# MiloszKrajewski/lz4net

Measured on AMD Instinct MI355X. Metric: uncompressed GB/s, batched 64KiB-block encode+decode: value = decode (known output size) per step over the whole resident batch; fast encode and LZ4HC encode of the same data in roofline_encode / roofline_hc, higher is better.
Workload: dtype u8

## Files before the change

### lz4net_amd/csrc/lz4hip_decode_lane4.hpp

```cpp
#pragma once
#include "lz4hip_common.hpp"
#include <type_traits>

#ifndef LZ4HIP_ITERATION_HOOK
#define LZ4HIP_ITERATION_HOOK(lane) ((void)0)
#endif
#ifndef LZ4HIP_STAT
#define LZ4HIP_STAT(slot, cond) ((void)0)
#endif
#ifdef LZ4HIP_SECTION_MARKERS
#define LZ4HIP_SECTION(name) asm volatile("; @@SECTION " name)
#else
#define LZ4HIP_SECTION(name) ((void)0)
#endif

namespace lz4hip {

#ifndef LZ4HIP_DEC4_FLUSH_RECS
#define LZ4HIP_DEC4_FLUSH_RECS 0
#endif
#ifndef LZ4HIP_DEC4_DUAL_STORE
#define LZ4HIP_DEC4_DUAL_STORE 2
#endif
constexpr unsigned lane4_lds_bytes(int ring_bytes) { return 64u * (unsigned)ring_bytes + 16u * 32u; }

struct NoNext {
    static constexpr bool kPersistent = false;
    LZ4HIP_DEVICE bool operator()(int, const uint8_t*&, int&, uint8_t*&, int&) const { return false; }
};

enum L4Kind { kK4None = 0, kK4Near = 1, kK4Far = 2, kK4Lit = 3, kK4Zero = 4 };
enum L4Flag { kF4Final = 1, kF4Err = 2, kF4Header = 4 };

template <bool KNOWN, int R, int P, int FU, int FS, int FE = 1, int IE = 1, int POL = 0, class NEXT = NoNext, int WAVES = 1>
LZ4HIP_DEVICE int lane4_decode_block(unsigned char* lds, int lane, bool active, const uint8_t* src, int iend,
                                     uint8_t* dst, int oend, NEXT next = NEXT(), int wave = 0)
{
    static_assert(WAVES == 1 || WAVES == 4, "one or four wavefronts per workgroup");
    constexpr uint32_t kRow = 256u * (uint32_t)WAVES;
    static_assert(R >= 128 && R % 16 == 0 && R <= 1008, "ring: a multiple of 16 bytes, 128 .. 1008");
    static_assert(P == 32 || P == 64, "input piece: 32 or 64 bytes");
    static_assert(FU == 64 || (FU == 128 && R >= 192), "flush unit: 64 bytes, or 128 with a ring of at least 192");
    static_assert(FS == 1 || FS == 2, "one or two flush store instructions per iteration");
    static_assert(FE == 1 || FE == 2, "the flush runs in every iteration or in every second one");
    static_assert(IE == 1 || (IE == 2 && FE == 2), "input requests in every iteration, or alternating with the flush");
    constexpr int RW = R / 4;
    constexpr bool RPOW2 = (RW & (RW - 1)) == 0;
    constexpr uint32_t kRingBytes = (uint32_t)RW * kRow;
    constexpr uint32_t kLdsBytes = lane4_lds_bytes(R) * (uint32_t)WAVES;
    constexpr bool LS = (POL & 16) != 0;
    constexpr int kDual = (POL & 32) ? 0 : (LZ4HIP_DEC4_DUAL_STORE);
    static_assert(!LS || P == 32, "sector input feeds 32-byte pieces");
    constexpr int SK = LS ? 64 : P;
    constexpr int NW = 4 + P / 4, NL = LS ? 4 : P / 16;
    constexpr int HPR = FU / 16, RECS_PER_STORE = 64 / HPR;
    constexpr int kFlushRecs = (LZ4HIP_DEC4_FLUSH_RECS) ? (LZ4HIP_DEC4_FLUSH_RECS) : FS * RECS_PER_STORE;
    constexpr bool kLineNoWrap = R % 64 == 0;
    constexpr int kNearMax = R - 20;
    unsigned char* const frec_base = lds + kRingBytes + (uint32_t)wave * 256u;
    auto frec = [&](int i) -> Aligned16* {
        if (kFlushRecs <= 16) return (Aligned16*)(frec_base + (uint32_t)i * 16u);
        return (Aligned16*)(frec_base + (uint32_t)(i >> 4) * kRow + (uint32_t)(i & 15) * 16u);
    };
    const uint32_t lane4 = (uint32_t)(wave * 64 + lane) << 2;

    auto ring_add = [](uint32_t a, uint32_t rows256) -> uint32_t {
        const uint32_t t = a + rows256;
        if (RPOW2) return t & (kRingBytes - 1u);
        const uint32_t u = t - kRingBytes;
        return u < t ? u : t;
    };
#define L4_RING(a) (*(uint32_t*)(lds + (a)))
#define L4_PHASE_SEL(p_) wv::alignbyte(0x07060504u, 0x03020100u, (uint32_t)(p_) & 3u)

    int skew = 0, in_total = 0;
    uint64_t src_al = 0;
    uint32_t out_limit = 0;
    int ip = 0;
    uint32_t W[NW];
    wv::u32x4 L[NL];
    int wb = -16;
    int lvalid = 0;
    int pend_a = 0, pend_b = 0;
    int op = 0, fl = 0;
    uint32_t oa = lane4;
    int kind = kK4None, rem = 0, off = 8;
    int gready = 0;
    int pv = 0, p_ll = 0, p_st = 0, p_ml = 0, p_off = 0, p_flags = 0, p_res = 0;
    uint32_t p_l0 = 0, p_l1 = 0, p_l2 = 0;
    int hdr = 0;
    uint32_t token = 0;
    int final_seen = 0, final_run = 0, result = 0, done = 0;
    int exhausted = 0;
    wv::u32x4 fa = { 0, 0, 0, 0 }, fb = { 0, 0, 0, 0 };
#if defined(LZ4HIP_DEC4_BALLAST_VALU) || defined(LZ4HIP_DEC4_BALLAST_LDS)
    uint32_t ballast = 0;
#endif
#pragma unroll
    for (int j = 0; j < NW; j++) W[j] = 0;
#pragma unroll
    for (int j = 0; j < NL; j++) L[j] = wv::u32x4{ 0, 0, 0, 0 };
    auto start_block = [&](bool act) {
        skew = (int)((uint64_t)src & (uint64_t)(SK - 1));
        src_al = (uint64_t)src - (uint64_t)skew;
        in_total = iend > 0 ? (int)(((int64_t)skew + iend + P - 1) & ~(int64_t)(P - 1)) : 0;
        out_limit = oend > kLastLiterals ? (uint32_t)(oend - kLastLiterals) : 0u;
        ip = 0; wb = -16 - P; lvalid = 0; pend_a = 0; pend_b = 0; op = 0; fl = 0; oa = lane4;
        kind = kK4None; rem = 0; off = 8; gready = 0;
        pv = 0; p_ll = 0; p_st = 0; p_ml = 0; p_off = 0; p_flags = 0; p_res = 0; hdr = 0; token = 0;
        final_seen = 0; final_run = 0; result = 0; done = 0;
        if (!act || (!KNOWN && iend == 0)) { done = 1; final_seen = 1; }
    };
    start_block(active);

#define L4_STORE2(OFF_, v_) do { const uint32_t w_ = (v_); wv::lds_store_drop<OFF_>(lds, kLdsBytes, oa, w_); wv::lds_store_drop<OFF_>(lds, kLdsBytes, ob_, w_); } while (0)
#define L4_APPEND(d0_, d1_, d2_, d3_, n_, FOUR_)                                                         \
    do {                                                                                                \
        const uint32_t sb_ = (uint32_t)op & 3u;                                                         \
        const uint32_t s_ = wv::alignbyte(0x08070605u, 0x04030201u, sb_ ^ 3u);                          \
        wv::lds_mskor(&L4_RING(oa), 0xFFFFFFFFu << (8u * sb_), wv::perm(d0_, 0u, s_));                  \
        if (kDual) {                                                                                    \
                                                    \
            const uint32_t ob_ = oa - kRingBytes;                                                       \
            const uint32_t w1_ = wv::perm(d1_, d0_, s_), w2_ = wv::perm(d2_, d1_, s_);                  \
            if (kDual == 2) {                                         \
                wv::lds_store2_rows_drop<1 * WAVES, 2 * WAVES>(lds, kLdsBytes, oa, w1_, w2_);           \
                wv::lds_store2_rows_drop<1 * WAVES, 2 * WAVES>(lds, kLdsBytes, ob_, w1_, w2_);          \
                if (FOUR_) {                                                                            \
                    const uint32_t w3_ = wv::perm(d3_, d2_, s_), w4_ = wv::perm(0u, d3_, s_);           \
                    wv::lds_store2_rows_drop<3 * WAVES, 4 * WAVES>(lds, kLdsBytes, oa, w3_, w4_);       \
                    wv::lds_store2_rows_drop<3 * WAVES, 4 * WAVES>(lds, kLdsBytes, ob_, w3_, w4_);      \
                } else {                                                                                \
                    L4_STORE2(3 * kRow, wv::perm(0u, d2_, s_));                                         \
                }                                                                                       \
            } else {                                                                                    \
                L4_STORE2(kRow, w1_);                                                                   \
                L4_STORE2(2 * kRow, w2_);                                                               \
                if (FOUR_) {                                                                            \
                    L4_STORE2(3 * kRow, wv::perm(d3_, d2_, s_));                                        \
                    L4_STORE2(4 * kRow, wv::perm(0u, d3_, s_));                                         \
                } else {                                                                                \
                    L4_STORE2(3 * kRow, wv::perm(0u, d2_, s_));                                         \
                }                                                                                       \
            }                                                                                           \
        } else {                                                                                        \
            const uint32_t a1_ = ring_add(oa, kRow), a2_ = ring_add(oa, 2 * kRow), a3_ = ring_add(oa, 3 * kRow); \
            L4_RING(a1_) = wv::perm(d1_, d0_, s_);                                                      \
            L4_RING(a2_) = wv::perm(d2_, d1_, s_);                                                      \
            if (FOUR_) {                                                                                \
                L4_RING(a3_) = wv::perm(d3_, d2_, s_);                                                  \
                L4_RING(ring_add(oa, 4 * kRow)) = wv::perm(0u, d3_, s_);                                \
            } else {                                                                                    \
                L4_RING(a3_) = wv::perm(0u, d2_, s_);                                                   \
            }                                                                                           \
        }                                                                                               \
        oa = ring_add(oa, (((sb_ + (uint32_t)(n_)) << 6) & 0x700u) * (uint32_t)WAVES);                  \
        op += (n_);                                                                                     \
    } while (0)

    auto iteration = [&](auto flush_tag, wv::u32x4& ldF, wv::u32x4& usF, int& ld_pend, int& us_pend) __attribute__((always_inline)) -> bool {
        constexpr bool FLUSH = decltype(flush_tag)::value;
        constexpr bool INPUT = IE == 1 || !FLUSH;
        constexpr int kVm = (FLUSH ? FS : 0) + 1 + (INPUT ? NL : 0);
        LZ4HIP_ITERATION_HOOK(lane);
        LZ4HIP_SECTION("T1a window refill");
        int d = ip + skew - wb;
        {
            const bool no_more = wb + 16 + P >= in_total;
            const bool cross = (d >= P) & ((lvalid != 0) | no_more);
            const wv::mask_t cm = wv::cond(d >= P) & (wv::cond(lvalid != 0) | wv::cond(no_more));
#pragma unroll
            for (int j = 0; j < 4; j++) W[j] = wv::sel(cm, W[P / 4 + j], W[j]);
            if constexpr (LS) {
                const bool hi_half = ((wb + 16 + P) & 32) != 0;
                const wv::mask_t hm = wv::cond(((wb + 16 + P) & 32) != 0);
#pragma unroll
                for (int j = 0; j < 2; j++) {
                    W[4 + 4 * j] = wv::sel(cm, wv::sel(hm, L[2 + j].x, L[j].x), W[4 + 4 * j]); W[5 + 4 * j] = wv::sel(cm, wv::sel(hm, L[2 + j].y, L[j].y), W[5 + 4 * j]);
                    W[6 + 4 * j] = wv::sel(cm, wv::sel(hm, L[2 + j].z, L[j].z), W[6 + 4 * j]); W[7 + 4 * j] = wv::sel(cm, wv::sel(hm, L[2 + j].w, L[j].w), W[7 + 4 * j]);
                }
                lvalid = (cross & hi_half) ? 0 : lvalid;
            } else {
#pragma unroll
                for (int j = 0; j < NL; j++) {
                    W[4 + 4 * j] = wv::sel(cm, L[j].x, W[4 + 4 * j]); W[5 + 4 * j] = wv::sel(cm, L[j].y, W[5 + 4 * j]);
                    W[6 + 4 * j] = wv::sel(cm, L[j].z, W[6 + 4 * j]); W[7 + 4 * j] = wv::sel(cm, L[j].w, W[7 + 4 * j]);
                }
                lvalid = cross ? 0 : lvalid;
            }
            wb += cross ? P : 0;
            d -= cross ? P : 0;
        }
        LZ4HIP_SECTION("T1b cursor view (select tree + rotation)");
        const bool staged16 = d < P;
        LZ4HIP_STAT(0, true); LZ4HIP_STAT(1, done == 0); LZ4HIP_STAT(2, (done == 0) & !staged16);
        uint32_t x0, x1, x2, x3;
        {
            const uint32_t k = (uint32_t)d >> 2;
            uint32_t t[NW];
#pragma unroll
            for (int j = 0; j < NW; j++) t[j] = W[j];
            int n = NW;
#pragma unroll
            for (int sh = P / 8; sh >= 1; sh >>= 1) {
                const wv::mask_t m = wv::cond((k & (uint32_t)sh) != 0u);
                n -= sh;
#pragma unroll
                for (int j = 0; j < NW; j++)
                    if (j < n) t[j] = wv::sel(m, t[j + sh], t[j]);
            }
            const uint32_t sx = L4_PHASE_SEL(d);
            x0 = wv::perm(t[1], t[0], sx); x1 = wv::perm(t[2], t[1], sx); x2 = wv::perm(t[3], t[2], sx); x3 = wv::perm(t[4], t[3], sx);
        }
        LZ4HIP_SECTION("T1c near-match source rows");
        uint32_t v0, v1, v2, v3;
        {
            const uint32_t offn = kind == kK4Near ? (uint32_t)off : 4u;
            const uint32_t back = (((offn + 3u - ((uint32_t)op & 3u)) << 6) & ~0xFFu) * (uint32_t)WAVES;
            uint32_t sa;
            if (RPOW2) sa = (oa - back) & (kRingBytes - 1u);
            else { const uint32_t t = oa - back, u = t + kRingBytes; sa = u < t ? u : t; }
            const uint32_t r0 = L4_RING(sa), r1 = L4_RING(ring_add(sa, kRow)), r2 = L4_RING(ring_add(sa, 2 * kRow)),
                           r3 = L4_RING(ring_add(sa, 3 * kRow)), r4 = L4_RING(ring_add(sa, 4 * kRow));
            const uint32_t sr = L4_PHASE_SEL((uint32_t)op - offn);
            v0 = wv::perm(r1, r0, sr); v1 = wv::perm(r2, r1, sr); v2 = wv::perm(r3, r2, sr); v3 = wv::perm(r4, r3, sr);
        }

        LZ4HIP_SECTION("T2 cooperative flush");
        if constexpr (FLUSH) {
            const bool need = (done == 0) & (op - fl >= FU);
            const uint64_t needy = wv::ballot(need);
            const int cnt_all = wv::popc64(needy);
            const bool go = cnt_all != 0;
            int cnt = 0;
            bool mine = false;
            if (go) {
                cnt = cnt_all < kFlushRecs ? cnt_all : kFlushRecs;
                const int frank = wv::rank_below(needy);
                mine = need & (frank < kFlushRecs);
                if (mine) {
                    const uint64_t dp = (uint64_t)dst;
                    *frec(frank) = Aligned16{ { ring_add(oa, kRingBytes - ((((uint32_t)(op - fl)) << 6) & ~0xFFu) * (uint32_t)WAVES), (uint32_t)fl, (uint32_t)dp, (uint32_t)(dp >> 32) } };
                }
                wv::mem_sync();
            }
            const int sub = lane % HPR;
#pragma unroll
            for (int base = 0; base < FS * RECS_PER_STORE; base += RECS_PER_STORE) {
                const int idx = base + lane / HPR;
                const bool act = idx < cnt;
                const wv::mask_t act_m = wv::cond(idx < cnt);
                uint64_t g = 0;
                uint32_t q0 = 0, q1 = 0, q2 = 0, q3 = 0;
                if (act) {
                    const Aligned16 r = *frec(idx);
                    g = ((uint64_t)r.w[2] | ((uint64_t)r.w[3] << 32)) + (uint64_t)(r.w[1] + 16u * (uint32_t)sub);
                    const uint32_t b0 = ring_add(r.w[0], 4u * kRow * (uint32_t)sub);
                    if (kLineNoWrap) { q0 = L4_RING(b0); q1 = L4_RING(b0 + kRow); q2 = L4_RING(b0 + 2 * kRow); q3 = L4_RING(b0 + 3 * kRow); }
                    else { q0 = L4_RING(b0); q1 = L4_RING(ring_add(b0, kRow)); q2 = L4_RING(ring_add(b0, 2 * kRow)); q3 = L4_RING(ring_add(b0, 3 * kRow)); }
                }
                wv::vm_store16_mask(act_m, g, q0, q1, q2, q3);
            }
            LZ4HIP_STAT(3, need); LZ4HIP_STAT(4, need & !mine);
            if (go) {
                wv::mem_sync();
                fl += mine ? FU : 0;
            }
        }
        LZ4HIP_SECTION("T3 chunk size");
        const bool room = op - fl <= R - 46;
        const bool near = kind == kK4Near, lit = kind == kK4Lit;
        const bool can = room & (rem > 0) & !((kind == kK4Far) & (gready == 0)) & !(lit & !staged16);
        const int stride = (near & (off < 16)) ? off : 16;
        int n = can ? (rem < stride ? rem : stride) : 0;
        n = ((kind == kK4Zero) & (n > 8)) ? 8 : n;
        LZ4HIP_STAT(5, (done == 0) & (rem > 0)); LZ4HIP_STAT(6, (done == 0) & (rem > 0) & (n == 0)); LZ4HIP_STAT(7, (done == 0) & (rem > 0) & !room);
        LZ4HIP_STAT(8, (done == 0) & (rem > 0) & (kind == kK4Far) & (gready == 0)); LZ4HIP_STAT(9, (done == 0) & (rem > n));
        const int rem_after = rem - n;
        const int op_end = op + rem;

        LZ4HIP_SECTION("T4 parse ahead");
        const bool may_parse = (pv == 0) & (final_seen == 0) & !(lit & (rem > 0)) & staged16;
        LZ4HIP_STAT(10, may_parse); LZ4HIP_STAT(11, (done == 0) & (pv != 0));
        if (may_parse) {
            const uint32_t tok = hdr ? token : (x0 & 255u);
            const uint32_t t4 = tok >> 4, b1 = (x0 >> 8) & 255u, mlc = tok & 15u;
            const bool e1 = (hdr == 0) & (t4 == 15u), e2 = mlc == 15u;
            const int ll = hdr ? 0 : (int)t4 + (e1 ? (int)b1 : 0);
            const bool in_win = (hdr != 0) | (t4 <= 11u);
            const int o = hdr ? 0 : 1 + (int)t4;
            uint32_t ot;
            {
                const uint32_t q = (uint32_t)o >> 2;
                const wv::mask_t m1 = wv::cond((q & 1u) != 0u), m2 = wv::cond((q & 2u) != 0u);
                const uint32_t lo = wv::sel(m2, wv::sel(m1, x3, x2), wv::sel(m1, x1, x0));
                const uint32_t hi = wv::sel(m2, x3, wv::sel(m1, x2, x1));
                ot = wv::alignbyte(hi, lo, (uint32_t)o & 3u);
            }
            const int vo = (int)(ot & 0xFFFFu);
            const uint32_t extb = (ot >> 16) & 255u;
            const int ml = (int)mlc + kMinMatch + (e2 ? (int)extb : 0);
            const int lit_end = op_end + ll;
            const int p_after = ip + o + 2;
            bool trap = (ip + 16 > iend) | (e1 & (b1 == 255u)) | (ip + 1 + (e1 ? 1 : 0) + ll > iend);
            trap |= in_win & ((e2 & (extb == 255u)) | (vo > lit_end) | ((uint32_t)lit_end + (uint32_t)ml > out_limit));
            if (KNOWN) trap |= (hdr == 0) & (lit_end > oend - 8);
            else       trap |= ((hdr == 0) & ((lit_end > oend - kMfLimit) | (ip + 1 + (e1 ? 1 : 0) + ll > iend - 8))) | (in_win & e2 & !(p_after < iend - (kLastLiterals + 1)));
            p_l0 = wv::alignbyte(x1, x0, 1); p_l1 = wv::alignbyte(x2, x1, 1); p_l2 = wv::alignbyte(x3, x2, 1);
            token = tok;
            p_ll = in_win ? ll : 0;
            p_st = in_win ? 0 : ll;
            p_ml = in_win ? ml : 0;
            p_off = vo;
            p_flags = in_win ? 0 : (int)kF4Header;
            const int ip_fast = in_win ? p_after + (e2 ? 1 : 0) : ip + 1 + (e1 ? 1 : 0);
            if (trap) {
                LZ4HIP_SECTION("T4x byte-wise parser (trap)");
                int err = 0, pos = ip;
                if (!hdr) {
                    const uint32_t tk = ip < iend ? src[ip] : 0u;
                    int l = (int)(tk >> 4);
                    pos = ip + 1;
                    if (l == 15) {
                        uint32_t b = 255;
                        if (KNOWN) { do { b = pos < iend ? src[pos] : 0u; pos++; l += (int)b; if (l > (1 << 30)) { err = -pos; l = 0; break; } } while (b == 255); }
                        else       { while (pos < iend && b == 255) { b = src[pos]; pos++; l += (int)b; l = l > (1 << 30) ? (1 << 30) : l; } }
                    }
                    token = tk;
                    const int le = (int)((int64_t)op_end + l > 0x7FFFFFFF ? 0x7FFFFFFF : op_end + l);
                    const bool last = KNOWN ? (le > oend - 8) : ((le > oend - kMfLimit) | (pos + l > iend - 8));
                    p_ll = 0; p_st = l; p_ml = 0; p_off = 8;
                    if (last) {
                        if (KNOWN) { if (err == 0 && (le != oend || pos + l > iend)) err = -pos; }
                        else       { if (le > oend || pos + l != iend) err = -pos; }
                        p_flags = kF4Final;
                        p_res = KNOWN ? pos + l : le;
                        final_seen = 1;
                    } else {
                        if (KNOWN && err == 0 && pos + l > iend) err = -pos;
                        p_flags = kF4Header;
                    }
                    ip = pos;
                } else {
                    int p = ip;
                    const int o_ = (int)((p < iend ? src[p] : 0u) | ((p + 1 < iend ? src[p + 1] : 0u) << 8));
                    p += 2;
                    int m = (int)(token & 15u);
                    if (m == 15) {
                        if (KNOWN) {
                            uint32_t b;
                            while ((b = (p < iend ? src[p] : 0u)) == 255) { m += 255; p++; if (m > (1 << 30)) { err = -p; break; } }
                            m += (int)b; p++;
                        } else {
                            while (p < iend - (kLastLiterals + 1)) { const uint32_t b = src[p]; p++; m += (int)b; m = m > (1 << 30) ? (1 << 30) : m; if (b != 255) break; }
                        }
                    }
                    m += kMinMatch;
                    if (err != 0) {}
                    else if (op_end - o_ < 0) err = -(ip + 2);
                    else if ((int64_t)op_end + m > (int64_t)oend - kLastLiterals) err = -p;
                    p_ll = 0; p_st = 0; p_ml = m; p_off = o_; p_flags = 0;
                    ip = p;
                    hdr = 0;
                }
                if (err != 0) { p_flags = kF4Err; p_res = err; }
                hdr = (p_flags & kF4Header) ? 1 : 0;
            } else {
                ip = ip_fast;
                hdr = in_win ? 0 : 1;
            }
            LZ4HIP_SECTION("T4 parse ahead");
            pv = 1;
        }

        LZ4HIP_SECTION("T5 far fetch");
        {
            const wv::mask_t m_rem0 = wv::cond(rem_after == 0);
            const wv::mask_t f_cont = wv::cond(kind == kK4Far) & ~m_rem0;
            const wv::mask_t f_first = m_rem0 & wv::cond(op - fl <= R - 46) & wv::cond(pv != 0) & wv::cond(p_ml != 0) & wv::cond(p_flags == 0) & wv::cond(p_off > kNearMax);
            const int f_pos = (int)wv::sel(f_cont, (uint32_t)(op + n - off), (uint32_t)(op_end + p_ll - p_off));
            const wv::mask_t f_want = f_cont | f_first;
            const wv::mask_t f_do = f_want & wv::cond(f_pos + 16 <= fl);
            wv::vm_load16_mask<POL & 3>(f_do, (uint64_t)dst + (uint64_t)(uint32_t)f_pos, ldF);
            gready = (int)wv::sel(f_do, 1u, 0u);
            LZ4HIP_STAT(15, gready != 0); LZ4HIP_STAT(16, wv::sel(f_want & ~f_do, 1u, 0u) != 0u);
        }

        LZ4HIP_SECTION("T6 input request");
        if constexpr (INPUT) {
            const int lpos = wb + 16 + P;
            const wv::mask_t req = wv::cond((done | lvalid | us_pend) == 0) & wv::cond(lpos < in_total);
            const uint64_t g = src_al + (uint64_t)(uint32_t)lpos;
            wv::vm_load16_mask_off<(POL >> 2) & 3, 0>(req, g, L[0]);
            wv::vm_load16_mask_off<(POL >> 2) & 3, 16>(req, g, L[1]);
            if constexpr (NL == 4) {
                wv::vm_load16_mask_off<(POL >> 2) & 3, 32>(req, g, L[2]);
                wv::vm_load16_mask_off<(POL >> 2) & 3, 48>(req, g, L[3]);
            }
            ld_pend = (int)wv::sel(req, 1u, 0u);
        } else {
            ld_pend = 0;
        }

        LZ4HIP_SECTION("B1 wait");
        wv::vm_wait_list<kVm>(usF, L);
        lvalid = us_pend ? 1 : lvalid;
        us_pend = 0;

#if defined(LZ4HIP_DEC4_BALLAST_VALU) || defined(LZ4HIP_DEC4_BALLAST_LDS)
#ifdef LZ4HIP_DEC4_BALLAST_VALU
#pragma unroll
        for (int bi = 0; bi < LZ4HIP_DEC4_BALLAST_VALU; bi++) asm volatile("v_add_u32 %0, %0, %1" : "+v"(ballast) : "v"(lane4));
#endif
#ifdef LZ4HIP_DEC4_BALLAST_LDS
#pragma unroll
        for (int bi = 0; bi < LZ4HIP_DEC4_BALLAST_LDS; bi++) wv::lds_store_drop<0>(lds, kLdsBytes, 0x80000000u + lane4, ballast);
#endif
#endif
        LZ4HIP_SECTION("B3 chunk append");
        {
            const bool far_src = kind == kK4Far;
            v0 = lit ? x0 : (far_src ? usF.x : v0);
            v1 = lit ? x1 : (far_src ? usF.y : v1);
            v2 = lit ? x2 : (far_src ? usF.z : v2);
            v3 = lit ? x3 : (far_src ? usF.w : v3);
            if ((kind == kK4Zero) & (n > 0)) {
                uint64_t acc = 0;
                for (int b = 0; b < n; b++) acc |= (uint64_t)dst[op + b] << (8 * b);
                v0 = (uint32_t)acc; v1 = (uint32_t)(acc >> 32);
            }
            ip += lit ? n : 0;
            L4_APPEND(v0, v1, v2, v3, n, true);
            rem = rem_after;
            off = (near & (off < 16) & (n > 0)) ? off * 2 : off;
            kind = rem == 0 ? (int)kK4None : kind;
        }

        LZ4HIP_SECTION("B4 promote + literal append");
        {
            const bool promote = (rem == 0) & (pv != 0) & room;
            LZ4HIP_STAT(12, promote); LZ4HIP_STAT(13, (done == 0) & (rem == 0) & (pv != 0) & !room); LZ4HIP_STAT(14, (done == 0) & (rem == 0) & (pv == 0));
            const bool perr = promote & ((p_flags & kF4Err) != 0);
            const bool pgo = promote & !perr;
            L4_APPEND(p_l0, p_l1, p_l2, 0u, pgo ? p_ll : 0, false);
            if (perr) {
                done = 1; final_seen = 1; final_run = 0; result = p_res;
            }
            if (pgo) {
                const bool streamed = p_st > 0;
                rem = streamed ? p_st : p_ml;
                off = streamed ? off : p_off;
                kind = streamed ? (int)kK4Lit : (p_ml == 0 ? (int)kK4None : (p_off == 0 ? (int)kK4Zero : (p_off <= kNearMax ? (int)kK4Near : (int)kK4Far)));
                final_run = (p_flags & kF4Final) ? 1 : final_run;
                result = (p_flags & kF4Final) ? p_res : result;
            }
            pv = promote ? 0 : pv;
        }

        LZ4HIP_SECTION("B5 end of block + loop");
        if (final_run && rem == 0 && !pv && !done) {
            uint32_t qa = ring_add(oa, kRingBytes - ((((uint32_t)(op - fl)) << 6) & ~0xFFu) * (uint32_t)WAVES);
            while (op - fl >= 4) { const uint32_t qd = L4_RING(qa); __builtin_memcpy(dst + fl, &qd, 4); fl += 4; qa = ring_add(qa, kRow); }
            if (fl < op) {
                const uint32_t qd = L4_RING(qa);
                for (int b = 0; fl + b < op; b++) dst[fl + b] = (uint8_t)(qd >> (8 * b));
            }
            done = 1;
        }
        return !wv::any(done == 0);
    };

    for (;;) {
        if (!std::remove_reference<NEXT>::type::kPersistent) {
            if (iteration(std::true_type{}, fa, fb, pend_a, pend_b)) break;
            if (iteration(std::integral_constant<bool, FE == 1>{}, fb, fa, pend_b, pend_a)) break;
        } else {
            (void)iteration(std::true_type{}, fa, fb, pend_a, pend_b);
            (void)iteration(std::integral_constant<bool, FE == 1>{}, fb, fa, pend_b, pend_a);
            const bool fin = (done != 0) & (exhausted == 0);
            if (wv::any(fin)) {
                if (fin) {
                    if (next(result, src, iend, dst, oend)) start_block(true);
                    else exhausted = 1;
                }
                if (!wv::any(exhausted == 0)) break;
            }
        }
    }
    return result;
#undef L4_RING
#undef L4_PHASE_SEL
#undef L4_APPEND
#undef L4_STORE2
}

__global__ void __launch_bounds__(256) count_selected_kernel(Batch b, int filter, unsigned* count)
{
    unsigned mine = 0;
    for (int64_t blk = (int64_t)blockIdx.x * 256 + threadIdx.x; blk < b.n_blocks; blk += (int64_t)gridDim.x * 256)
        mine += block_selected(filter, batch_src_len(b, blk), batch_dst_cap(b, blk)) ? 1u : 0u;
    const unsigned total = wv::scan_add(mine);
    if ((threadIdx.x & 63u) == 63u && total) atomicAdd(count, total);
}
LZ4HIP_DEVICE bool lane4_gate_open(const unsigned* gate, int gate_mode, unsigned threshold)
{
    if (gate_mode == 0) return true;
    const unsigned c = wv::uniform(*gate);
    return gate_mode == 1 ? c >= threshold : c < threshold;
}

__global__ void __launch_bounds__(64) lds_drop_probe_kernel(unsigned* errors, int rounds)
{
    constexpr uint32_t kBytes = lane4_lds_bytes(192), kRing = 64u * 192u, kWords = kBytes / 4u;
    LZ4HIP_STATIC_LDS(lds, kBytes);
    uint32_t* const s = (uint32_t*)lds;
    const uint32_t lane = threadIdx.x, tag = 0x9E3779B9u * (blockIdx.x + 1u);
    for (uint32_t i = lane; i < kWords; i += 64u) s[i] = tag ^ i;
    wv::block_sync();
    for (int r = 0; r < rounds; r++) {
        const uint32_t junk = 0xDEAD0000u | (uint32_t)r;
        const uint32_t last = kRing - 256u + lane * 4u;
        const uint32_t own = tag ^ (last >> 2);
        wv::lds_store2_rows_drop<0, 3>(lds, kBytes, last, own, junk);
        wv::lds_store2_rows_drop<3, 4>(lds, kBytes, last, junk, junk);
        wv::lds_store_drop<1024>(lds, kBytes, last, junk);
        wv::lds_store_drop<768>(lds, kBytes, kBytes - 256u + lane * 4u, junk);
        const uint32_t neg = lane * 4u - kRing;
        wv::lds_store2_rows_drop<1, 2>(lds, kBytes, neg, junk, junk);
        wv::lds_store2_rows_drop<3, 4>(lds, kBytes, neg + 2048u, junk, junk);
        wv::lds_store_drop<768>(lds, kBytes, neg, junk);
        wv::lds_store2_rows_drop<0, 48>(lds, kBytes, neg, junk, tag ^ lane);
        wv::mem_sync();
#if defined(__HIP_DEVICE_COMPILE__)
        __builtin_amdgcn_s_sleep(8);
#endif
    }
    wv::block_sync();
    unsigned bad = 0;
    for (uint32_t i = lane; i < kWords; i += 64u) bad += s[i] != (tag ^ i) ? 1u : 0u;
    if (bad) atomicAdd(errors, bad);
}

template <bool KNOWN, int R, int P, int FU, int FS, int FE = 1, int IE = 1, int POL = 0>
__global__ void __launch_bounds__(64) decode_lane4_kernel(Batch b, int filter, const unsigned* gate = nullptr, int gate_mode = 0, unsigned threshold = 0)
{
    LZ4HIP_STATIC_LDS(lds, lane4_lds_bytes(R));
    if (!lane4_gate_open(gate, gate_mode, threshold)) return;
    const int lane = (int)threadIdx.x;
    const int64_t blk = (int64_t)blockIdx.x * 64 + lane;
    bool active = blk < b.n_blocks;
    int src_len = 0, out_size = 0;
    if (active) {
        src_len = batch_src_len(b, blk); out_size = batch_dst_cap(b, blk);
        active = block_selected(filter, src_len, out_size);
    }
    if (!wv::any(active)) return;
    const uint8_t* src = active ? batch_src(b, blk) : nullptr;
    uint8_t* dst = active ? batch_dst(b, blk) : nullptr;
    const int r = lane4_decode_block<KNOWN, R, P, FU, FS, FE, IE, POL>(lds, lane, active, src, src_len, dst, out_size);
    if (active) b.result[blk] = r;
}

template <bool KNOWN, int R, int P, int FU, int FS, int FE = 1, int IE = 1, int POL = 0>
__global__ void __launch_bounds__(256) decode_lane4_wg4_kernel(Batch b, int filter)
{
    LZ4HIP_STATIC_LDS(lds_all, 4u * lane4_lds_bytes(R));
    const int lane = (int)(threadIdx.x & 63u);
    const int w = wv::wave_in_block();
    const int64_t blk = ((int64_t)blockIdx.x * 4 + w) * 64 + lane;
    bool active = blk < b.n_blocks;
    int src_len = 0, out_size = 0;
    if (active) {
        src_len = batch_src_len(b, blk); out_size = batch_dst_cap(b, blk);
        active = block_selected(filter, src_len, out_size);
    }
    if (!wv::any(active)) return;
    const uint8_t* src = active ? batch_src(b, blk) : nullptr;
    uint8_t* dst = active ? batch_dst(b, blk) : nullptr;
    const int r = lane4_decode_block<KNOWN, R, P, FU, FS, FE, IE, POL, NoNext, 4>(lds_all, lane, active, src, src_len, dst, out_size, NoNext(), w);
    if (active) b.result[blk] = r;
}

struct PullNext {
    static constexpr bool kPersistent = true;
    const Batch* b; int filter; unsigned long long* counter; int64_t cur;
    LZ4HIP_DEVICE bool operator()(int r, const uint8_t*& src, int& iend, uint8_t*& dst, int& oend)
    {
        if (cur >= 0) b->result[cur] = r;
        for (;;) {
            const int64_t blk = (int64_t)atomicAdd(counter, 1ull);
            if (blk >= b->n_blocks) { cur = -1; return false; }
            const int sl = batch_src_len(*b, blk), oc = batch_dst_cap(*b, blk);
            if (!block_selected(filter, sl, oc)) continue;
            cur = blk; src = batch_src(*b, blk); iend = sl; dst = batch_dst(*b, blk); oend = oc;
            return true;
        }
    }
};

template <bool KNOWN, int R, int P, int FU, int FS, int FE = 1, int IE = 1, int POL = 0>
__global__ void __launch_bounds__(64) decode_lane4_persistent_kernel(Batch b, int filter, unsigned long long* counter, const unsigned* gate = nullptr,
                                                                     int gate_mode = 0, unsigned threshold = 0)
{
    LZ4HIP_STATIC_LDS(lds, lane4_lds_bytes(R));
    if (!lane4_gate_open(gate, gate_mode, threshold)) return;
    const int lane = (int)threadIdx.x;
    PullNext next{ &b, filter, counter, -1 };
    const uint8_t* src = nullptr; uint8_t* dst = nullptr; int src_len = 0, out_size = 0;
    const bool active = next(0, src, src_len, dst, out_size);
    if (!wv::any(active)) return;
    (void)lane4_decode_block<KNOWN, R, P, FU, FS, FE, IE, POL, PullNext&>(lds, lane, active, src, src_len, dst, out_size, next);
}

}
```

Before: 1043.

## Split cooperative flush into phases interleaved with window refill and parse

Breaks the per-iteration cooperative flush into record publish, record read, ring-row LDS reads and global stores, and spreads these across the iteration. Near-match LDS reads are hoisted before the window refill and cursor select tree, so LDS latency and the flush's memory syncs can overlap with ALU work. The ring-row reads now run unconditionally with a fallback address for inactive lanes, and the flush stores move after the parse step. This raises register pressure because all FS records and row values stay live across T3/T4, and it adds section begin/end hooks for profiling.

```diff
diff --git a/lz4net_amd/csrc/lz4hip_decode_lane4.hpp b/lz4net_amd/csrc/lz4hip_decode_lane4.hpp
--- a/lz4net_amd/csrc/lz4hip_decode_lane4.hpp
+++ b/lz4net_amd/csrc/lz4hip_decode_lane4.hpp
@@ -10,8 +10,12 @@
 #endif
 #ifdef LZ4HIP_SECTION_MARKERS
 #define LZ4HIP_SECTION(name) asm volatile("; @@SECTION " name)
-#else
+#elif !defined(LZ4HIP_SECTION)
 #define LZ4HIP_SECTION(name) ((void)0)
+#endif
+#ifndef LZ4HIP_SECTION_BEGIN
+#define LZ4HIP_SECTION_BEGIN() ((void)0)
+#define LZ4HIP_SECTION_END(lane) ((void)0)
 #endif
 
 namespace lz4hip {
@@ -112,6 +116,7 @@
         if (!act || (!KNOWN && iend == 0)) { done = 1; final_seen = 1; }
     };
     start_block(active);
+    LZ4HIP_SECTION_BEGIN();
 
 #define L4_STORE2(OFF_, v_) do { const uint32_t w_ = (v_); wv::lds_store_drop<OFF_>(lds, kLdsBytes, oa, w_); wv::lds_store_drop<OFF_>(lds, kLdsBytes, ob_, w_); } while (0)
 #define L4_APPEND(d0_, d1_, d2_, d3_, n_, FOUR_)                                                         \
@@ -163,76 +168,18 @@
         constexpr bool INPUT = IE == 1 || !FLUSH;
         constexpr int kVm = (FLUSH ? FS : 0) + 1 + (INPUT ? NL : 0);
         LZ4HIP_ITERATION_HOOK(lane);
-        LZ4HIP_SECTION("T1a window refill");
-        int d = ip + skew - wb;
-        {
-            const bool no_more = wb + 16 + P >= in_total;
-            const bool cross = (d >= P) & ((lvalid != 0) | no_more);
-            const wv::mask_t cm = wv::cond(d >= P) & (wv::cond(lvalid != 0) | wv::cond(no_more));
-#pragma unroll
-            for (int j = 0; j < 4; j++) W[j] = wv::sel(cm, W[P / 4 + j], W[j]);
-            if constexpr (LS) {
-                const bool hi_half = ((wb + 16 + P) & 32) != 0;
-                const wv::mask_t hm = wv::cond(((wb + 16 + P) & 32) != 0);
-#pragma unroll
-                for (int j = 0; j < 2; j++) {
-                    W[4 + 4 * j] = wv::sel(cm, wv::sel(hm, L[2 + j].x, L[j].x), W[4 + 4 * j]); W[5 + 4 * j] = wv::sel(cm, wv::sel(hm, L[2 + j].y, L[j].y), W[5 + 4 * j]);
-                    W[6 + 4 * j] = wv::sel(cm, wv::sel(hm, L[2 + j].z, L[j].z), W[6 + 4 * j]); W[7 + 4 * j] = wv::sel(cm, wv::sel(hm, L[2 + j].w, L[j].w), W[7 + 4 * j]);
-                }
-                lvalid = (cross & hi_half) ? 0 : lvalid;
-            } else {
-#pragma unroll
-                for (int j = 0; j < NL; j++) {
-                    W[4 + 4 * j] = wv::sel(cm, L[j].x, W[4 + 4 * j]); W[5 + 4 * j] = wv::sel(cm, L[j].y, W[5 + 4 * j]);
-                    W[6 + 4 * j] = wv::sel(cm, L[j].z, W[6 + 4 * j]); W[7 + 4 * j] = wv::sel(cm, L[j].w, W[7 + 4 * j]);
-                }
-                lvalid = cross ? 0 : lvalid;
-            }
-            wb += cross ? P : 0;
-            d -= cross ? P : 0;
-        }
-        LZ4HIP_SECTION("T1b cursor view (select tree + rotation)");
-        const bool staged16 = d < P;
-        LZ4HIP_STAT(0, true); LZ4HIP_STAT(1, done == 0); LZ4HIP_STAT(2, (done == 0) & !staged16);
-        uint32_t x0, x1, x2, x3;
-        {
-            const uint32_t k = (uint32_t)d >> 2;
-            uint32_t t[NW];
-#pragma unroll
-            for (int j = 0; j < NW; j++) t[j] = W[j];
-            int n = NW;
-#pragma unroll
-            for (int sh = P / 8; sh >= 1; sh >>= 1) {
-                const wv::mask_t m = wv::cond((k & (uint32_t)sh) != 0u);
-                n -= sh;
-#pragma unroll
-                for (int j = 0; j < NW; j++)
-                    if (j < n) t[j] = wv::sel(m, t[j + sh], t[j]);
-            }
-            const uint32_t sx = L4_PHASE_SEL(d);
-            x0 = wv::perm(t[1], t[0], sx); x1 = wv::perm(t[2], t[1], sx); x2 = wv::perm(t[3], t[2], sx); x3 = wv::perm(t[4], t[3], sx);
-        }
-        LZ4HIP_SECTION("T1c near-match source rows");
-        uint32_t v0, v1, v2, v3;
-        {
-            const uint32_t offn = kind == kK4Near ? (uint32_t)off : 4u;
-            const uint32_t back = (((offn + 3u - ((uint32_t)op & 3u)) << 6) & ~0xFFu) * (uint32_t)WAVES;
-            uint32_t sa;
-            if (RPOW2) sa = (oa - back) & (kRingBytes - 1u);
-            else { const uint32_t t = oa - back, u = t + kRingBytes; sa = u < t ? u : t; }
-            const uint32_t r0 = L4_RING(sa), r1 = L4_RING(ring_add(sa, kRow)), r2 = L4_RING(ring_add(sa, 2 * kRow)),
-                           r3 = L4_RING(ring_add(sa, 3 * kRow)), r4 = L4_RING(ring_add(sa, 4 * kRow));
-            const uint32_t sr = L4_PHASE_SEL((uint32_t)op - offn);
-            v0 = wv::perm(r1, r0, sr); v1 = wv::perm(r2, r1, sr); v2 = wv::perm(r3, r2, sr); v3 = wv::perm(r4, r3, sr);
-        }
-
-        LZ4HIP_SECTION("T2 cooperative flush");
+        LZ4HIP_SECTION("T2a flush records");
+        bool go = false;
+        int cnt = 0;
+        wv::mask_t f_act_m[FS];
+        Aligned16 f_rec[FS];
+        uint64_t f_g[FS];
+        uint32_t f_q[FS][4];
         if constexpr (FLUSH) {
             const bool need = (done == 0) & (op - fl >= FU);
             const uint64_t needy = wv::ballot(need);
             const int cnt_all = wv::popc64(needy);
-            const bool go = cnt_all != 0;
-            int cnt = 0;
+            go = cnt_all != 0;
             bool mine = false;
             if (go) {
                 cnt = cnt_all < kFlushRecs ? cnt_all : kFlushRecs;
@@ -242,31 +189,87 @@
                     const uint64_t dp = (uint64_t)dst;
                     *frec(frank) = Aligned16{ { ring_add(oa, kRingBytes - ((((uint32_t)(op - fl)) << 6) & ~0xFFu) * (uint32_t)WAVES), (uint32_t)fl, (uint32_t)dp, (uint32_t)(dp >> 32) } };
                 }
-                wv::mem_sync();
-            }
-            const int sub = lane % HPR;
-#pragma unroll
-            for (int base = 0; base < FS * RECS_PER_STORE; base += RECS_PER_STORE) {
-                const int idx = base + lane / HPR;
-                const bool act = idx < cnt;
-                const wv::mask_t act_m = wv::cond(idx < cnt);
-                uint64_t g = 0;
-                uint32_t q0 = 0, q1 = 0, q2 = 0, q3 = 0;
-                if (act) {
-                    const Aligned16 r = *frec(idx);
-                    g = ((uint64_t)r.w[2] | ((uint64_t)r.w[3] << 32)) + (uint64_t)(r.w[1] + 16u * (uint32_t)sub);
-                    const uint32_t b0 = ring_add(r.w[0], 4u * kRow * (uint32_t)sub);
-                    if (kLineNoWrap) { q0 = L4_RING(b0); q1 = L4_RING(b0 + kRow); q2 = L4_RING(b0 + 2 * kRow); q3 = L4_RING(b0 + 3 * kRow); }
-                    else { q0 = L4_RING(b0); q1 = L4_RING(ring_add(b0, kRow)); q2 = L4_RING(ring_add(b0, 2 * kRow)); q3 = L4_RING(ring_add(b0, 3 * kRow)); }
+                fl += mine ? FU : 0;
+            }
+            LZ4HIP_STAT(3, need); LZ4HIP_STAT(4, need & !mine);
+        }
+        LZ4HIP_SECTION("T2b record read");
+        if constexpr (FLUSH) {
+            if (go) wv::mem_sync();
+#pragma unroll
+            for (int s = 0; s < FS; s++) {
+                const int idx = s * RECS_PER_STORE + lane / HPR;
+                f_act_m[s] = wv::cond(idx < cnt);
+                f_rec[s] = *frec(idx);
+            }
+        }
+        LZ4HIP_SECTION("T1c near-match reads");
+        const uint32_t offn = kind == kK4Near ? (uint32_t)off : 4u;
+        uint32_t r0, r1, r2, r3, r4;
+        {
+            const uint32_t back = (((offn + 3u - ((uint32_t)op & 3u)) << 6) & ~0xFFu) * (uint32_t)WAVES;
+            uint32_t sa;
+            if (RPOW2) sa = (oa - back) & (kRingBytes - 1u);
+            else { const uint32_t t = oa - back, u = t + kRingBytes; sa = u < t ? u : t; }
+            r0 = L4_RING(sa); r1 = L4_RING(ring_add(sa, kRow)); r2 = L4_RING(ring_add(sa, 2 * kRow));
+            r3 = L4_RING(ring_add(sa, 3 * kRow)); r4 = L4_RING(ring_add(sa, 4 * kRow));
+        }
+        LZ4HIP_SECTION("T1a window refill");
+        int d = ip + skew - wb;
+        {
+            const bool no_more = wb + 16 + P >= in_total;
+            const bool cross = (d >= P) & ((lvalid != 0) | no_more);
+            const wv::mask_t cm = wv::cond(d >= P) & (wv::cond(lvalid != 0) | wv::cond(no_more));
+#pragma unroll
+            for (int j = 0; j < 4; j++) W[j] = wv::sel(cm, W[P / 4 + j], W[j]);
+            if constexpr (LS) {
+                const bool hi_half = ((wb + 16 + P) & 32) != 0;
+                const wv::mask_t hm = wv::cond(((wb + 16 + P) & 32) != 0);
+#pragma unroll
+                for (int j = 0; j < 2; j++) {
+                    W[4 + 4 * j] = wv::sel(cm, wv::sel(hm, L[2 + j].x, L[j].x), W[4 + 4 * j]); W[5 + 4 * j] = wv::sel(cm, wv::sel(hm, L[2 + j].y, L[j].y), W[5 + 4 * j]);
+                    W[6 + 4 * j] = wv::sel(cm, wv::sel(hm, L[2 + j].z, L[j].z), W[6 + 4 * j]); W[7 + 4 * j] = wv::sel(cm, wv::sel(hm, L[2 + j].w, L[j].w), W[7 + 4 * j]);
                 }
-                wv::vm_store16_mask(act_m, g, q0, q1, q2, q3);
-            }
-            LZ4HIP_STAT(3, need); LZ4HIP_STAT(4, need & !mine);
-            if (go) {
-                wv::mem_sync();
-                fl += mine ? FU : 0;
-            }
-        }
+                lvalid = (cross & hi_half) ? 0 : lvalid;
+            } else {
+#pragma unroll
+                for (int j = 0; j < NL; j++) {
+                    W[4 + 4 * j] = wv::sel(cm, L[j].x, W[4 + 4 * j]); W[5 + 4 * j] = wv::sel(cm, L[j].y, W[5 + 4 * j]);
+                    W[6 + 4 * j] = wv::sel(cm, L[j].z, W[6 + 4 * j]); W[7 + 4 * j] = wv::sel(cm, L[j].w, W[7 + 4 * j]);
+                }
+                lvalid = cross ? 0 : lvalid;
+            }
+            wb += cross ? P : 0;
+            d -= cross ? P : 0;
+        }
+        LZ4HIP_SECTION("T1b cursor view (select tree + rotation)");
+        const bool staged16 = d < P;
+        LZ4HIP_STAT(0, true); LZ4HIP_STAT(1, done == 0); LZ4HIP_STAT(2, (done == 0) & !staged16);
+        uint32_t x0, x1, x2, x3;
+        {
+            const uint32_t k = (uint32_t)d >> 2;
+            uint32_t t[NW];
+#pragma unroll
+            for (int j = 0; j < NW; j++) t[j] = W[j];
+            int n = NW;
+#pragma unroll
+            for (int sh = P / 8; sh >= 1; sh >>= 1) {
+                const wv::mask_t m = wv::cond((k & (uint32_t)sh) != 0u);
+                n -= sh;
+#pragma unroll
+                for (int j = 0; j < NW; j++)
+                    if (j < n) t[j] = wv::sel(m, t[j + sh], t[j]);
+            }
+            const uint32_t sx = L4_PHASE_SEL(d);
+            x0 = wv::perm(t[1], t[0], sx); x1 = wv::perm(t[2], t[1], sx); x2 = wv::perm(t[3], t[2], sx); x3 = wv::perm(t[4], t[3], sx);
+        }
+        LZ4HIP_SECTION("T1c near-match source rows");
+        uint32_t v0, v1, v2, v3;
+        {
+            const uint32_t sr = L4_PHASE_SEL((uint32_t)op - offn);
+            v0 = wv::perm(r1, r0, sr); v1 = wv::perm(r2, r1, sr); v2 = wv::perm(r3, r2, sr); v3 = wv::perm(r4, r3, sr);
+        }
+
         LZ4HIP_SECTION("T3 chunk size");
         const bool room = op - fl <= R - 46;
         const bool near = kind == kK4Near, lit = kind == kK4Lit;
@@ -278,6 +281,19 @@
         LZ4HIP_STAT(8, (done == 0) & (rem > 0) & (kind == kK4Far) & (gready == 0)); LZ4HIP_STAT(9, (done == 0) & (rem > n));
         const int rem_after = rem - n;
         const int op_end = op + rem;
+
+        LZ4HIP_SECTION("T2c ring rows");
+        if constexpr (FLUSH) {
+            const int sub = lane % HPR;
+#pragma unroll
+            for (int s = 0; s < FS; s++) {
+                const Aligned16 r = f_rec[s];
+                f_g[s] = ((uint64_t)r.w[2] | ((uint64_t)r.w[3] << 32)) + (uint64_t)(r.w[1] + 16u * (uint32_t)sub);
+                const uint32_t b0 = wv::sel(f_act_m[s], ring_add(r.w[0], 4u * kRow * (uint32_t)sub), lane4);
+                if (kLineNoWrap) { f_q[s][0] = L4_RING(b0); f_q[s][1] = L4_RING(b0 + kRow); f_q[s][2] = L4_RING(b0 + 2 * kRow); f_q[s][3] = L4_RING(b0 + 3 * kRow); }
+                else { f_q[s][0] = L4_RING(b0); f_q[s][1] = L4_RING(ring_add(b0, kRow)); f_q[s][2] = L4_RING(ring_add(b0, 2 * kRow)); f_q[s][3] = L4_RING(ring_add(b0, 3 * kRow)); }
+            }
+        }
 
         LZ4HIP_SECTION("T4 parse ahead");
         const bool may_parse = (pv == 0) & (final_seen == 0) & !(lit & (rem > 0)) & staged16;
@@ -373,6 +389,13 @@
             pv = 1;
         }
 
+        LZ4HIP_SECTION("T2d flush stores");
+        if constexpr (FLUSH) {
+#pragma unroll
+            for (int s = 0; s < FS; s++) wv::vm_store16_mask(f_act_m[s], f_g[s], f_q[s][0], f_q[s][1], f_q[s][2], f_q[s][3]);
+            if (go) wv::mem_sync();
+        }
+
         LZ4HIP_SECTION("T5 far fetch");
         {
             const wv::mask_t m_rem0 = wv::cond(rem_after == 0);
@@ -487,6 +510,7 @@
             }
         }
     }
+    LZ4HIP_SECTION_END(lane);
     return result;
 #undef L4_RING
 #undef L4_PHASE_SEL
```

New measurement: 1054, median of 6. +1.0%, better.
